# liuyuan-pal/NeuRay

Measured on AMD Instinct MI355X. Metric: rays/sec (64 coarse+32 fine samples), lego 800x800 synthetic, higher is better.
Workload: dtype fp32 (MLP contractions: operands split exactly into 3 bf16 parts, 6 bf16-MFMA products per K = 32, fp32 accumulate); 1 GPU; lego-800 synthetic (nerf_synthetic/lego/black_800 shape): 800x800 = 640000 rays/image, 8 ref views, 64 coarse + 32 fine samples, maps 200x200x32, 1 image per step per GPU; ray_batch=65536, parallelism=images sharded over 1 GPU(s), no collective

## Files before the change

__graft_entry__.py:

```python
import os
import subprocess
import sys

ROOT = os.path.dirname(os.path.abspath(__file__))
if ROOT not in sys.path:
    sys.path.insert(0, ROOT)


def build():
    from concurrent.futures import ThreadPoolExecutor
    from neuray_amd import build as nbuild
    sys.path.insert(0, os.path.join(ROOT, 'tests', 'emu'))
    import build_emu
    with ThreadPoolExecutor(4) as pool:
        jobs = [pool.submit(nbuild.build, False, True)]
        jobs += [pool.submit(build_emu.build, False, variant) for variant in ('fp32', 'bf16', 'bf16x3')]
        for j in jobs:
            j.result()
    from neuray_amd import _lib
    lib = _lib.bind(_lib.LIB_PATH)
    assert lib.neuray_abi_version() == 11 and lib.neuray_is_device_build() == 1 and lib.neuray_operand_precision() == 32
    import neuray_amd.network.renderer


def smoke():
    import numpy as np
    import torch
    from oracle import neuray_oracle as orc
    from neuray_amd.network.renderer import NeuralRayBaseRenderer

    assert torch.cuda.is_available(), "smoke() needs the MI355X"
    dev = 'cuda:0'
    cfg = {'use_hierarchical_sampling': True, 'dist_decoder_cfg': {'use_vis': False}, 'depth_sample_num': 32,
           'fine_depth_sample_num': 32, 'agg_net_cfg': {'sample_num': 32}, 'fine_agg_net_cfg': {'sample_num': 32}}
    torch.manual_seed(0)
    r = NeuralRayBaseRenderer(cfg).eval()
    weights = {k: v.detach().numpy().copy() for k, v in r.state_dict().items()}
    r = r.to(dev)
    que, ref = orc.make_scene(96, 128, 4, seed=7)
    rng = np.random.RandomState(7)
    que['coords'] = (rng.rand(1, 96, 2) * np.array([127, 95])).astype(np.float32)
    tq = {k: torch.from_numpy(v).to(dev) for k, v in que.items()}
    tr = {k: torch.from_numpy(v).to(dev) for k, v in ref.items()}
    with torch.no_grad():
        got = r.render_impl(tq, tr, False)
    torch.cuda.synchronize()
    ocfg = dict(cfg, coarse_use_vis=False, fine_use_vis=True)
    want = orc.render_impl(weights, ocfg, dict(que, Ks_inv=torch.inverse(torch.from_numpy(que['Ks'])).numpy()), ref)
    err_c = float(np.abs(got['pixel_colors_nr'].cpu().numpy() - want['pixel_colors_nr']).max())
# ... 59 lines not shown
```

include/neuray_hip.h:

```cpp
#ifndef NEURAY_HIP_H
#define NEURAY_HIP_H

#include <stddef.h>

#ifdef __cplusplus
extern "C" {
#endif

#define NEURAY_ABI_VERSION 11
#define NEURAY_POINT_REC 20
#define NEURAY_VIEW_CONST 20
#define NEURAY_QUERY_CONST 28
#define NEURAY_PASS_TENSORS 68
#define NEURAY_DBG_FIELDS 16
#define NEURAY_MAX_VIEWS 16
#define NEURAY_MAX_SAMPLES 128

int neuray_abi_version(void);
const char* neuray_last_error(void);
int neuray_is_device_build(void);
int neuray_operand_precision(void);

size_t neuray_packed_pass_floats(void);
int neuray_pack_pass_weights(const float* const* tensors_host, float* packed_host);
// ... 223 lines not shown
long long neuray_lpips_head_workspace_bytes(int n, int h, int w);
int neuray_lpips_head(const float* f0_dev, const float* f1_dev, const float* lin_dev, int n, int f1_stride, int c, int h, int w,
                      void* workspace_dev, double* out_dev, int out_stride, void* stream);

#define NEURAY_LOSS_RENDER 0
#define NEURAY_LOSS_CONSIST 1
#define NEURAY_LOSS_DEPTH 2
#define NEURAY_LOSS_MAX_TERMS 4
typedef struct NeurayLossTerm {
    const float* pred_dev;
    const float* ref_dev;
    const void* mask_dev;
    const void* coords_dev;
    const float* range_dev;
    const float* grad_out_dev;
    float* d_pred_dev;
    int kind, rows, n, inner, stride, h, w, coords_i64, mask_u8, smooth_l1;
    float beta, thresh;
} NeurayLossTerm;
typedef struct NeurayTrainLossArgs {
    const NeurayLossTerm* terms;
    float* value_dev;
    double* den_dev;
    void* workspace_dev;
    int n_terms, reserved;
} NeurayTrainLossArgs;
long long neuray_train_loss_workspace_bytes(const NeurayLossTerm* terms, int n_terms);
int neuray_train_loss(const NeurayTrainLossArgs* args, void* stream);
int neuray_train_loss_backward(const NeurayTrainLossArgs* args, void* stream);

int neuray_mfma_selftest(const float* A_dev, const float* B_dev, float* D_dev, void* stream);
int neuray_group_sum_selftest(const float* x_dev, float* y_dev, void* stream);
int neuray_group_scatter_selftest(const float* x_dev, float* y_dev, void* stream);

int neuray_x3_selftest(const float* A_dev, const float* B_dev, float* D_dev, float* parts_dev, void* stream);
int neuray_points_resident_workgroups(int arith, int rfn);

#ifdef __cplusplus
}
#endif
#endif
```

neuray_amd/_lib.py:

```python
import ctypes as C
import os

import torch

HERE = os.path.dirname(os.path.abspath(__file__))
LIB_PATH = os.environ.get('NEURAY_HIP_LIB', os.path.join(HERE, 'libneuray_hip.so'))
BF16_LIB_PATH = os.path.join(HERE, 'libneuray_hip_bf16.so')
BF16X3_LIB_PATH = os.path.join(HERE, 'libneuray_hip_bf16x3.so')

PASS_TENSORS = 68
POINT_REC = 20
VIEW_CONST = 20
QUERY_CONST = 28
DBG_FIELDS = 16
MAX_VIEWS = 16
MAX_SAMPLES = 128
MAX_BACKWARD_SAMPLES = 128

ARITH_F32, ARITH_X3 = 0, 1

c_float_p = C.POINTER(C.c_float)


class NeurayPointsArgs(C.Structure):
# ... 107 lines not shown
    'neuray_inorm_backward': (C.c_int, [C.c_void_p, C.c_void_p, C.c_longlong, C.c_void_p, C.c_longlong, C.c_void_p, C.c_void_p] + [C.c_int] * 6 + [C.c_void_p] * 6),
    'neuray_upsample2x_pad_forward': (C.c_int, [C.c_void_p, C.c_int, C.c_int, C.c_int, C.c_int, C.c_float, C.c_float, C.c_void_p, C.c_void_p]),
    'neuray_upsample2x_pad_backward': (C.c_int, [C.c_void_p, C.c_int, C.c_int, C.c_int, C.c_int, C.c_void_p, C.c_void_p, C.c_void_p, C.c_void_p,
                                                 C.c_void_p, C.c_void_p, C.c_void_p, C.c_void_p]),
    'neuray_direct_render_points': (C.c_int, [C.c_void_p] * 7 + [C.c_int] * 5 + [C.c_float, C.c_void_p, C.c_void_p, C.c_void_p]),
    'neuray_direct_render_rays': (C.c_int, [C.c_void_p, C.c_void_p, C.c_int, C.c_int, C.c_int, C.c_int, C.c_void_p, C.c_void_p, C.c_void_p]),
    'neuray_direct_render_rays_backward': (C.c_int, [C.c_void_p] * 4 + [C.c_int] * 2 + [C.c_void_p] * 3),
    'neuray_direct_render_points_backward': (C.c_int, [C.c_void_p] * 9 + [C.c_int] * 6 + [C.c_void_p] * 2),
    'neuray_dist_decoder_rows': (C.c_int, [C.c_void_p, C.c_void_p, C.c_int, C.c_int, C.c_float, C.c_void_p, C.c_void_p, C.c_void_p,
                                           C.c_void_p, C.c_void_p]),
    'neuray_self_hit_prob': (C.c_int, [C.c_void_p, C.c_void_p, C.c_void_p, C.c_void_p, C.c_void_p, C.c_void_p, C.c_int, C.c_int,
                                       C.c_void_p, C.c_void_p]),
    'neuray_mfma_selftest': (C.c_int, [C.c_void_p, C.c_void_p, C.c_void_p, C.c_void_p]),
    'neuray_x3_selftest': (C.c_int, [C.c_void_p, C.c_void_p, C.c_void_p, C.c_void_p, C.c_void_p]),
    'neuray_points_resident_workgroups': (C.c_int, [C.c_int, C.c_int]),
    'neuray_render_rays_backward': (C.c_int, [C.POINTER(NeurayRaysBwdArgs), C.c_void_p]),
    'neuray_flat_pass_floats': (C.c_size_t, []),
    'neuray_flat_tensor_offset': (C.c_size_t, [C.c_int]),
    'neuray_packed_t_floats': (C.c_size_t, []),
    'neuray_pack_pass_t_index_map': (C.c_int, [C.c_int, C.c_void_p]),
    'neuray_points_backward_handover_floats': (C.c_size_t, [C.c_int]),
    'neuray_packed_quad_ranges': (C.c_int, [C.c_int, C.c_void_p, C.c_int]),
    'neuray_render_points_backward': (C.c_int, [C.POINTER(NeurayPointsBwdArgs), C.c_void_p]),
    'neuray_self_hit_prob_backward': (C.c_int, [C.c_void_p, C.c_void_p, C.c_void_p, C.c_void_p, C.c_void_p, C.c_int, C.c_int,
                                                         C.c_float, C.c_void_p, C.c_int, C.c_int, C.c_void_p, C.c_void_p, C.c_void_p]),
    'neuray_dist_decoder_rows_backward': (C.c_int, [C.c_void_p, C.c_void_p, C.c_void_p, C.c_int, C.c_int, C.c_float, C.c_void_p, C.c_void_p,
                                                           C.c_void_p, C.c_void_p, C.c_void_p, C.c_void_p, C.c_void_p]),
    'neuray_interpolate_feats_backward_staged': (C.c_int, [C.c_void_p, C.c_void_p, C.c_void_p, C.c_int, C.c_int, C.c_int, C.c_int, C.c_int, C.c_int,
                                                         C.c_int, C.c_int, C.c_void_p, C.c_void_p, C.c_void_p]),
    'neuray_interpolate_feats_backward': (C.c_int, [C.c_void_p, C.c_void_p, C.c_void_p, C.c_int, C.c_int, C.c_int, C.c_int,
                                                    C.c_int, C.c_int, C.c_int, C.c_int, C.c_void_p, C.c_void_p]),
    'neuray_group_sum_selftest': (C.c_int, [C.c_void_p, C.c_void_p, C.c_void_p]),
    'neuray_group_scatter_selftest': (C.c_int, [C.c_void_p, C.c_void_p, C.c_void_p]),
    'neuray_warp_variance': (C.c_int, [C.c_void_p, C.c_void_p, C.c_void_p, C.c_void_p, C.c_void_p, C.c_int, C.c_int, C.c_int, C.c_int, C.c_int,
                                       C.c_int, C.c_void_p, C.c_void_p]),
    'neuray_warp_variance_layout': (C.c_int, [C.c_void_p, C.c_void_p, C.c_void_p, C.c_void_p, C.c_void_p, C.c_int, C.c_int, C.c_int, C.c_int, C.c_int,
                                              C.c_int, C.c_int, C.c_void_p, C.c_void_p]),
    'neuray_conv3d_c32_c8': (C.c_int, [C.c_void_p, C.c_void_p, C.c_void_p, C.c_float, C.c_int, C.c_int, C.c_int, C.c_int, C.c_void_p, C.c_void_p]),
    'neuray_convtranspose3d_bn_leaky': (C.c_int, [C.c_void_p, C.c_void_p, C.c_void_p, C.c_float, C.c_void_p, C.c_int, C.c_int, C.c_int, C.c_int, C.c_int,
                                                C.c_int, C.c_void_p, C.c_void_p]),
    'neuray_conv3d_bn_leaky': (C.c_int, [C.c_void_p, C.c_void_p, C.c_void_p, C.c_float, C.c_int, C.c_int, C.c_int, C.c_int, C.c_int, C.c_int, C.c_int,
                                       C.c_void_p, C.c_void_p]),
    'neuray_conv3x3_x3_pack_bytes': (C.c_longlong, [C.c_int, C.c_int]),
    'neuray_conv3x3_x3_pack': (C.c_int, [C.c_void_p, C.c_int, C.c_int, C.c_void_p, C.c_void_p, C.c_void_p]),
    'neuray_conv3x3_x3': (C.c_int, [C.c_void_p, C.c_void_p, C.c_void_p, C.c_int, C.c_int, C.c_int, C.c_int, C.c_int, C.c_int, C.c_void_p, C.c_void_p]),
    'neuray_conv3x3_x3_relu': (C.c_int, [C.c_void_p, C.c_void_p, C.c_void_p, C.c_int, C.c_int, C.c_int, C.c_int, C.c_int, C.c_int, C.c_void_p, C.c_void_p]),
    'neuray_conv3x3_x3_wrw_workspace_floats': (C.c_longlong, [C.c_int, C.c_int, C.c_int, C.c_int, C.c_int]),
    'neuray_conv3x3_x3_wrw': (C.c_int, [C.c_void_p, C.c_void_p, C.c_int, C.c_int, C.c_int, C.c_int, C.c_int, C.c_void_p, C.c_void_p, C.c_void_p]),
    'neuray_scale_shift_leaky': (C.c_int, [C.c_void_p, C.c_void_p, C.c_void_p, C.c_int, C.c_int, C.c_longlong, C.c_float, C.c_void_p]),
    'neuray_conv3d_c8_c1': (C.c_int, [C.c_void_p, C.c_void_p, C.c_float, C.c_int, C.c_int, C.c_int, C.c_int, C.c_void_p, C.c_void_p]),
    'neuray_convtranspose3d_c16_c8': (C.c_int, [C.c_void_p, C.c_void_p, C.c_void_p, C.c_float, C.c_void_p, C.c_int, C.c_int, C.c_int, C.c_int, C.c_void_p, C.c_void_p]),
    'neuray_diff_feats': (C.c_int, [C.c_void_p, C.c_void_p, C.c_void_p, C.c_int, C.c_int, C.c_int, C.c_void_p, C.c_void_p]),
    'neuray_image_metrics_workspace_bytes': (C.c_longlong, [C.c_int, C.c_int, C.c_int]),
    'neuray_image_metrics': (C.c_int, [C.POINTER(NeurayImageMetricsArgs), C.c_void_p]),
    'neuray_lpips_stem': (C.c_int, [C.c_void_p, C.c_int, C.POINTER(C.c_float), C.POINTER(C.c_float), C.c_void_p, C.c_void_p, C.c_int, C.c_int, C.c_int,
                                    C.c_int, C.c_void_p, C.c_void_p]),
    'neuray_maxpool2x2': (C.c_int, [C.c_void_p, C.c_longlong, C.c_int, C.c_int, C.c_void_p, C.c_void_p]),
    'neuray_lpips_head_workspace_bytes': (C.c_longlong, [C.c_int, C.c_int, C.c_int]),
    'neuray_lpips_head': (C.c_int, [C.c_void_p, C.c_void_p, C.c_void_p, C.c_int, C.c_int, C.c_int, C.c_int, C.c_int, C.c_void_p, C.c_void_p, C.c_int,
                                    C.c_void_p]),
    'neuray_train_loss_workspace_bytes': (C.c_longlong, [C.POINTER(NeurayLossTerm), C.c_int]),
    'neuray_train_loss': (C.c_int, [C.POINTER(NeurayTrainLossArgs), C.c_void_p]),
    'neuray_train_loss_backward': (C.c_int, [C.POINTER(NeurayTrainLossArgs), C.c_void_p]),
}


# ... 36 lines not shown
```

neuray_amd/build.py:

```python
import os
import subprocess
import sys

HERE = os.path.dirname(os.path.abspath(__file__))
CSRC = os.path.join(HERE, 'csrc')
OUT = os.path.join(HERE, 'libneuray_hip.so')
SOURCES = [os.path.join(CSRC, 'neuray_hip.hip'), os.path.join(CSRC, 'nr_pack.cpp')]
DEPS = SOURCES + [os.path.join(CSRC, f) for f in ('nr_kernels.h', 'nr_kernels_bwd.h', 'nr_kernels_bwd2.h', 'nr_kernels_dr.h', 'nr_kernels_norm.h', 'nr_kernels_conv3d.h', 'nr_kernels_conv2d.h', 'nr_kernels_metrics.h', 'nr_kernels_loss.h', 'nr_kernels_lpips.h', 'nr_device.h', 'nr_layout.h', 'nr_platform.h', 'nr_pack.h')] + \
    [os.path.join(os.path.dirname(HERE), 'include', 'neuray_hip.h')]
HIPCC = os.environ.get('HIPCC', '/opt/rocm/bin/hipcc')
FLAGS = ['--offload-arch=gfx950', '-O3', '-std=c++17', '-fPIC', '-shared', '-ffp-contract=off', '-Wno-unused-value', '-Wno-pass-failed',
         '-Wno-comment']


OUT_BF16 = os.path.join(HERE, 'libneuray_hip_bf16.so')
OUT_BF16X3 = os.path.join(HERE, 'libneuray_hip_bf16x3.so')


def needs_build(out=OUT):
    return not os.path.exists(out) or any(os.path.getmtime(out) < os.path.getmtime(d) for d in DEPS)


def build(force=False, verbose=False):
    jobs = []
    for out, extra in ((OUT, []), (OUT_BF16, ['-DNR_BF16_QUADS']), (OUT_BF16X3, ['-DNR_BF16_QUADS', '-DNR_BF16_SPLIT'])):
        if not force and not needs_build(out):
            continue
        tmp = out + '.building'
        cmd = [HIPCC] + FLAGS + extra + SOURCES + ['-o', tmp]
        if verbose:
            print(' '.join(cmd[:-1] + [out]))
        jobs.append((out, tmp, cmd, subprocess.Popen(cmd)))
    failed = []
    for out, tmp, cmd, proc in jobs:
        if proc.wait() == 0:
            os.replace(tmp, out)
        else:
            failed.append(cmd)
            if os.path.exists(tmp):
                os.remove(tmp)
    if failed:
        raise subprocess.CalledProcessError(1, failed[0])
    return OUT


if __name__ == '__main__':
    print(build(force='-f' in sys.argv, verbose=True))
```

neuray_amd/csrc/neuray_hip.hip:

```cpp
#include "nr_kernels.h"
#include "nr_kernels_bwd.h"
#include "nr_kernels_norm.h"
#include "nr_kernels_conv3d.h"
#include "nr_kernels_conv2d.h"
#include "nr_kernels_metrics.h"
#include "nr_kernels_loss.h"
#include "nr_kernels_lpips.h"
#if defined(NR_BF16_QUADS) && !defined(NR_BF16_SPLIT)
#define NR_INFERENCE_ONLY 1
#else
#include "nr_kernels_bwd2.h"
#endif
#include "nr_kernels_dr.h"
#include "nr_pack.h"
#include "../../include/neuray_hip.h"

#include <cmath>
#include <cstdarg>
#include <cstdio>
#include <cstring>
#include <cstdlib>

namespace {

// ... 857 lines not shown
    if (has_vis_head && d_vis) NR_LAUNCH(nr::decoder_rows_backward2_kernel<true>, grid, dim3(64), 0, stream, p);
    else NR_LAUNCH(nr::decoder_rows_backward2_kernel<false>, grid, dim3(64), 0, stream, p);
    return check_launch("neuray_dist_decoder_rows_backward");
#endif
}

int neuray_interpolate_feats_backward(const float* d_out, const float* points, const float* mask, int b, int n, int c, int fh,
                                      int fw, int h_full, int w_full, int align_corners, float* d_feats, void* stream) {
    if (!d_out || !points || !d_feats) return fail("neuray_interpolate_feats_backward: null argument");
    if (b < 1 || n < 1 || c < 1 || fh < 1 || fw < 1) return fail("neuray_interpolate_feats_backward: bad shape");
    NR_LAUNCH(nr::interpolate_backward_kernel, dim3(grid_for((long long)b * n * c, 256, 4096)), dim3(256), 0, stream, d_out, points,
              mask, b, n, c, fh, fw, h_full, w_full, align_corners, d_feats);
    return check_launch("neuray_interpolate_feats_backward");
}

int neuray_interpolate_feats_backward_staged(const float* d_out, const float* points, const float* mask, int b, int n, int c, int fh,
                                             int fw, int h_full, int w_full, int align_corners, float* tmp_nhwc_zeroed, float* d_feats, void* stream) {
    if (!d_out || !points || !d_feats || !tmp_nhwc_zeroed) return fail("neuray_interpolate_feats_backward_staged: null argument");
    if (b < 1 || n < 1 || c < 1 || fh < 1 || fw < 1 || (long long)b * ((c + 31) / 32) > 65535) return fail("neuray_interpolate_feats_backward_staged: bad shape");
    NR_LAUNCH(nr::interpolate_backward_nhwc_kernel, dim3(grid_for((long long)b * n * c, 256, 4096)), dim3(256), 0, stream, d_out, points,
              mask, b, n, c, fh, fw, h_full, w_full, align_corners, tmp_nhwc_zeroed);
    if (int rc = check_launch("neuray_interpolate_feats_backward_staged")) return rc;
    NR_LAUNCH(nr::nhwc_add_to_nchw_kernel, dim3((fh * fw + 31) / 32, ((c + 31) / 32) * b), dim3(256), 0, stream, tmp_nhwc_zeroed, fh * fw, c, d_feats);
    return check_launch("neuray_interpolate_feats_backward_staged");
}

int neuray_group_sum_selftest(const float* x, float* y, void* stream) {
    NR_LAUNCH(nr::group_sum_selftest_kernel, dim3(1), dim3(64), 0, stream, x, y);
    return check_launch("neuray_group_sum_selftest");
}
int neuray_group_scatter_selftest(const float* x, float* y, void* stream) {
    NR_LAUNCH(nr::group_scatter_selftest_kernel, dim3(1), dim3(64), 0, stream, x, y);
    return check_launch("neuray_group_scatter_selftest");
}

static void metrics_tiles(int y0, int y1, int x0, int x1, int& tiles_y, int& tiles_x) {
    tiles_y = (y1 - y0 - (nr::kMetWin - 1) + nr::kMetTH - 1) / nr::kMetTH;
    tiles_x = (x1 - x0 - (nr::kMetWin - 1) + nr::kMetTW - 1) / nr::kMetTW;
}

long long neuray_image_metrics_workspace_bytes(int n, int h, int w) {
    if (n < 1 || h < nr::kMetWin || w < nr::kMetWin) return -1;
    int ty, tx;
    metrics_tiles(0, h, 0, w, ty, tx);
    return (long long)n * ty * tx * nr::kMetPartial * 8;
}

int neuray_image_metrics(const NeurayImageMetricsArgs* a, void* stream) {
    if (!a) return fail("neuray_image_metrics: null args");
    if (!a->pred_dev || !a->gt_dev || !a->sse_dev || !a->ssim_dev || !a->workspace_dev) return fail("neuray_image_metrics: missing array");
    if (a->n < 1 || a->h < 1 || a->w < 1 || a->gt_stride < 0) return fail("neuray_image_metrics: bad shape n=%d h=%d w=%d gt_stride=%d", a->n, a->h, a->w, a->gt_stride);
    if (a->variant != NEURAY_SSIM_BOX11 && a->variant != NEURAY_SSIM_GAUSS11) return fail("neuray_image_metrics: unknown SSIM variant %d", a->variant);
    if (a->roi_y0 < 0 || a->roi_x0 < 0 || a->roi_y1 > a->h || a->roi_x1 > a->w || a->roi_y0 >= a->roi_y1 || a->roi_x0 >= a->roi_x1)
        return fail("neuray_image_metrics: region [%d, %d) x [%d, %d) is not inside the %d x %d image", a->roi_y0, a->roi_y1, a->roi_x0, a->roi_x1, a->h, a->w);
    if (a->roi_y1 - a->roi_y0 < nr::kMetWin || a->roi_x1 - a->roi_x0 < nr::kMetWin)
        return fail("neuray_image_metrics: the %d x %d region is smaller than the 11 x 11 SSIM window", a->roi_y1 - a->roi_y0, a->roi_x1 - a->roi_x0);
    nr::MetricsParams p;
    p.pred = a->pred_dev; p.gt = a->gt_dev; p.quant = a->quant_dev; p.sse = a->sse_dev; p.ssim = a->ssim_dev;
    p.ws = static_cast<double*>(a->workspace_dev);
    p.n = a->n; p.gt_stride = a->gt_stride; p.u8 = a->input_u8 ? 1 : 0; p.h = a->h; p.w = a->w;
    p.y0 = a->roi_y0; p.y1 = a->roi_y1; p.x0 = a->roi_x0; p.x1 = a->roi_x1;
    metrics_tiles(p.y0, p.y1, p.x0, p.x1, p.tiles_y, p.tiles_x);
    double sum = 0.0;
    for (int k = 0; k < nr::kMetWin; ++k) {
        const double d = k - (nr::kMetWin - 1) / 2;
        p.taps[k] = std::exp(-0.5 * d * d / (1.5 * 1.5));
// ... 149 lines not shown
```

neuray_amd/csrc/nr_kernels.h:

```cpp
#pragma once
#include "nr_device.h"

namespace nr {

__global__ void view_setup_kernel(const float* __restrict__ poses, const float* __restrict__ Ks,
                                  const float* __restrict__ depth_range, int n, float* __restrict__ out) {
    const int v = blockIdx.x * blockDim.x + threadIdx.x;
    if (v >= n) return;
    const float* P = poses + v * 12;
    const float* K = Ks + v * 9;
    float* o = out + v * kViewConst;
    for (int i = 0; i < 3; ++i)
        for (int j = 0; j < 4; ++j)
            o[i * 4 + j] = dot3(K[i * 3 + 0], K[i * 3 + 1], K[i * 3 + 2], P[j], P[4 + j], P[8 + j]);
    for (int i = 0; i < 3; ++i) o[12 + i] = dot3(-P[i], -P[4 + i], -P[8 + i], P[3], P[7], P[11]);
    o[15] = rn_div(-1.0f, depth_range[2 * v]);
    o[16] = rn_div(-1.0f, depth_range[2 * v + 1]);
    o[17] = rn_div(1.0f, rn_sub(o[16], o[15]));
    o[18] = 0.0f; o[19] = 0.0f;
}

__global__ void query_setup_kernel(const float* __restrict__ pose, const float* __restrict__ Kinv,
                                   const float* __restrict__ depth_range, float* __restrict__ o) {
    if (blockIdx.x * blockDim.x + threadIdx.x != 0) return;
// ... 117 lines not shown
        const int mo = wave + j * nw;
        if (mo < 4) {
            mfma_quad<NT>(r.q[j][2 * STAT], 0, xq, accg[j]);
            mfma_quad<NT>(r.q[j][2 * STAT + 1], 1, xq, accg[j]);
            NR_PRAGMA_UNROLL
            for (int t = 0; t < NT; ++t) accg[j][t] = nr_mfma16(r.s1[j][STAT], x1[t][0], accg[j][t]);
        }
    }
}

template <int NA, int IDLE, int R, int RMAX, int OP>
__device__ __forceinline__ void view_allreduce(const float (&v)[NA > 0 ? NA : 1][R], float (&out)[R], float* red, int wave,
                                               int nw, int lane) {
    NR_PRAGMA_UNROLL
    for (int r = 0; r < R; ++r) {
        const bool is_max = OP == RED_MAX || (OP == RED_MAX0 && r == 0);
        float a = NA > 0 ? v[0][r] : (is_max ? -1e9f : 0.0f);
        NR_PRAGMA_UNROLL
        for (int s = 1; s < NA; ++s) a = red_combine<OP, R>(a, v[s][r], r);
        if (IDLE > 0 && NA > 0 && is_max) a = fmaxf(a, -1e9f);
        out[r] = a;
    }
    block_allreduce<R, RMAX, OP, R>(out, red, wave, nw, lane);
}

template <int N> struct SlotCount { static constexpr int value = N; };

#ifndef NR_POINT_SKIP
#define NR_POINT_SKIP 1
#endif
#ifndef NR_POINT_TILE_ORDER
#define NR_POINT_TILE_ORDER 0
#endif
#ifndef NR_POINT_TRANSPOSED
#define NR_POINT_TRANSPOSED 1
#endif

template <int NT, int VPW, bool HAS_VIS, int OWN, int MAXT, int MINW, bool SAVE = false, bool DBG = false, int AR = AR_F32>
__global__ void __launch_bounds__(MAXT, MINW) points_kernel(PointParams p) {
    static_assert(NT == 1, "one 16-point tile per wave iteration");
    static_assert(AR == AR_F32 || !SAVE, "the training forward runs on the fp32 MFMA");
    NR_DYNAMIC_SMEM(float, smem);
    constexpr int RMAX = point_rmax<NT>();
    constexpr int NS = VPW;
    constexpr bool SKIP = (NR_POINT_SKIP != 0) && !SAVE && !DBG && VPW == 2;
    const int lane = threadIdx.x & 63;
    const int wave = NR_UNIFORM((int)(threadIdx.x >> 6));
    const int nw = (p.rfn + VPW - 1) / VPW;
    const int g = lane >> 4, c = lane & 15;
    float* red = smem;
    float* xch = smem + (size_t)(nw + 1) * RMAX * 64;
    float* wl = xch + (AR == AR_X3 ? 0 : 16 * NT * 64);
    auto xrow = [&](int mo, int r) -> float* {
        if constexpr (AR == AR_X3 && OWN == 1) return red + ((size_t)mo * RMAX + r) * 64;
        else if constexpr (AR == AR_X3) return red + ((size_t)(mo % nw) * RMAX + (mo / nw) * 4 + r) * 64;
        else return xch + (mo * 4 + r) * 64;
    };
    auto make_w = [&]() {
        if constexpr (AR == AR_X3) return GlbW3{nr_make_wbuf(p.weights, sizeof(float) * kPackedPointFloatsX3)};
        else return nr_make_wbuf(p.weights, sizeof(float) * kPackedPassFloats);
    };
    const auto W = make_w();
    const float w_m1 = (float)(p.w - 1), h_m1 = (float)(p.h - 1);
    const float inv_w_m1 = 1.0f / w_m1, inv_h_m1 = 1.0f / h_m1, inv_rfn = 1.0f / (float)p.rfn;
    const size_t fmap = (size_t)p.fh * p.fw * 32, imap = (size_t)p.h * p.w * 4;
    const nr_mbuf rf_map = nr_make_mbuf(p.ray_feats, sizeof(float) * fmap * p.rfn);
    const nr_mbuf if_map = nr_make_mbuf(p.img_feats, sizeof(float) * fmap * p.rfn);
    const nr_mbuf rgb_map = nr_make_mbuf(p.rgba, sizeof(float) * imap * p.rfn);
    const int goff = 32 * g;
    const int npts = p.rn * p.dn;
    const int dn = p.dn;
    const bool use_vis = p.use_vis != 0;
    const bool folded = AR == AR_X3 || (!SAVE && p.folded != 0);
    const int bid = (int)(blockIdx.x % 8) * (int)(gridDim.x / 8) + (int)(blockIdx.x / 8);
    int seq0 = 0;
#ifndef NR_X3_BG_RESIDENT
#define NR_X3_BG_RESIDENT 1
#endif
#ifndef NR_X3_GF_PREFETCH
#define NR_X3_GF_PREFETCH 1
#endif
    constexpr bool BG_RES = AR == AR_X3 && OWN == 1 && (NR_X3_BG_RESIDENT != 0);
    BgResident<OWN> bgres;
    if constexpr (BG_RES) bg_resident_load(W, lane, wave, nw, bgres);
    int n_active = 0, n_slots = 0;
    constexpr bool TR = (NR_POINT_TRANSPOSED != 0) && !SAVE && !DBG;
    const int nloop = TR ? ((p.rn + 15) / 16) * dn * 16 : npts;
#ifndef NR_POINT_CHUNK
#define NR_POINT_CHUNK 1
#endif
    constexpr int CH = NR_POINT_CHUNK;
    const int G = (int)gridDim.x;
    auto tile_base = [&](int it) { return (((it / CH) * G + bid) * CH + (it % CH)) * 16; };
    if (tile_base(0) < nloop) stage_issue<PH_DIST_M>(wl, W, wave, nw, lane);
    for (int it = 0, base; (base = tile_base(it)) < nloop; ++it, seq0 += phase_count(HAS_VIS)) {
        const bool more = tile_base(it + 1) < nloop;
        const int glane = lane + nr_opaque_zero();
#ifndef NR_NO_OPAQUE_WAVE
        const int wave_t = wave + nr_opaque_szero();
#else
        const int wave_t = wave;
#endif
        const int gg = glane >> 4;
        const bool dbg_lane = DBG && (gg == 0);
        const auto* pt = NR_ARGS_HERE(PointParams, p);
        int pidx; bool pvalid;
        float mask[NS], dlt[NS][4], tref[NS], pu[NS], pv[NS], lo, hi;
        int soff_f[NS], soff_c[NS];
        {
            int pi, ray, smp;
            const float* __restrict__ qc = pt->que_const;
            const float qnearp = qc[24], qfarp = qc[25], qinv = qc[27];
            const int dn = pt->dn, npts = pt->rn * dn;
            if constexpr (TR) {
#if NR_POINT_TILE_ORDER == 1
                const int tix = base >> 4, nrb = (pt->rn + 15) / 16;
                smp = tix / nrb;
                const int rb = tix - smp * nrb;
#else
                const int tix = base >> 4, rb = tix / dn;
                smp = tix - rb * dn;
#endif
                ray = rb * 16 + c;
                pvalid = ray < pt->rn;
                ray = pvalid ? ray : pt->rn - 1;
                pi = ray * dn + smp;
            } else {
                pi = base + c;
                pvalid = pi < npts;
                pi = pi < npts ? pi : npts - 1;
                ray = pi / dn;
                smp = pi - ray * dn;
            }
            pidx = pi;
            const Ray r = make_ray<false>(qc, pt->coords[2 * ray], pt->coords[2 * ray + 1]);
            const float* drow = pt->depth + (size_t)ray * dn;
            const float d = drow[smp];
            float s_c, s_n, s_p, s_x;
            {
                const int nxt = smp + 1 < dn ? smp + 1 : smp, prv = smp > 0 ? smp - 1 : 0;
                const float dg = drow[gg == 0 ? smp : (gg == 1 ? nxt : prv)];
                nr_group_gather4(norm_inv_depth_fast(dg, qnearp, qfarp, qinv), s_c, s_n, s_p, s_x);
            }
            const float half_c = (smp == dn - 1) ? 500000.0f : (s_n - s_c) * 0.5f;
            const float half_p = (s_c - s_p) * 0.5f;
            hi = half_c;
            lo = (smp == 0) ? half_c : half_p;
            const float px = rn_add(r.cx, rn_mul(r.dx, d));
            const float py = rn_add(r.cy, rn_mul(r.dy, d));
            const float pz = rn_add(r.cz, rn_mul(r.dz, d));
            NR_PRAGMA_UNROLL
            for (int s = 0; s < NS; ++s) {
                const int vraw = wave_t * VPW + s;
                const bool vok = vraw < pt->rfn;
                const int view = vok ? vraw : pt->rfn - 1;
                const float* __restrict__ vc = pt->view_const + view * kViewConst;
                Proj pr = project_point<false>(vc, px, py, pz, (float)pt->w, (float)pt->h);
                if (!vok) pr.mask = 0.0f;
                mask[s] = pr.mask;
                dlt[s][0] = pr.dirx - r.qx; dlt[s][1] = pr.diry - r.qy; dlt[s][2] = pr.dirz - r.qz;
                dlt[s][3] = dot3(pr.dirx, pr.diry, pr.dirz, r.qx, r.qy, r.qz);
                tref[s] = norm_inv_depth_fast(fmaxf(pr.z, 1e-5f), vc[15], vc[16], vc[17]);
                pu[s] = pr.u; pv[s] = pr.v;
                if (dbg_lane && pvalid && vok) {
                    float* d_ = pt->dbg + ((size_t)pi * pt->rfn + view) * kDbgFields;
                    d_[0] = pr.mask; d_[1] = pr.u; d_[2] = pr.v; d_[3] = pr.z;
                }
                soff_f[s] = view * (int)(fmap * sizeof(float)); soff_c[s] = view * (int)(imap * sizeof(float));
            }
        }

        auto tile = [&](auto na_tag) NR_LAMBDA_INLINE {
            constexpr int NA = decltype(na_tag)::value, NA1 = NA > 0 ? NA : 1, IDLE = NS - NA;
            constexpr bool SC = NA == 2 && !SAVE;
            float fray[NA1][8], fimg[NA1][8], rgb[NA1][3];
#ifdef NR_PROBE_PRE
            float fm1[NA1][8], fv1[NA1][8], fa1[NA1][8];
#endif
            if constexpr (NA > 0) {
                Taps tfs[NA], tcs[NA];
                NR_PRAGMA_UNROLL
                for (int s = 0; s < NA; ++s) {
                    tfs[s] = make_taps_fast(pu[s], pv[s], w_m1, h_m1, inv_w_m1, inv_h_m1, p.fw, p.fh, p.fw == p.w && p.fh == p.h);
                    tcs[s] = make_taps_fast(pu[s], pv[s], w_m1, h_m1, inv_w_m1, inv_h_m1, p.w, p.h, true);
#ifdef NR_PROBE_NO_GATHER
                    tfs[s].o00 = tfs[s].o10 = tfs[s].o01 = tfs[s].o11 = 0;
                    tcs[s].o00 = tcs[s].o10 = tcs[s].o01 = tcs[s].o11 = 0;
#endif
                }
                NR_PRAGMA_UNROLL
                for (int s = 0; s < NA; ++s) {
                    float4 qf[8], qi[8], qc4[4];
                    issue8(rf_map, goff, soff_f[s], tfs[s], qf);
                    issue8(if_map, goff, soff_f[s], tfs[s], qi);
                    issue_rgb(rgb_map, soff_c[s], tcs[s], qc4);
                    NR_PIN();
                    blend8(qf, tfs[s], mask[s], fray[s]);
                    blend8(qi, tfs[s], mask[s], fimg[s]);
                    blend_rgb(qc4, tcs[s], mask[s], rgb[s]);
                    NR_PRAGMA_UNROLL
                    for (int k = 0; k < 8; ++k) { NR_KEEP(fray[s][k]); NR_KEEP(fimg[s][k]); }
                    NR_PRAGMA_UNROLL
                    for (int j = 0; j < 3; ++j) NR_KEEP(rgb[s][j]);
                    NR_PIN();
#ifdef NR_PROBE_PRE
                    {
                        float4 q1[8], q2[8], q3[8];
                        issue8(rf_map, goff, soff_f[s] + 4096, tfs[s], q1);
                        issue8(rf_map, goff, soff_f[s] + 8192, tfs[s], q2);
                        issue8(rf_map, goff, soff_f[s] + 12288, tfs[s], q3);
                        NR_PIN();
                        blend8(q1, tfs[s], mask[s], fm1[s]);
                        blend8(q2, tfs[s], mask[s], fv1[s]);
                        blend8(q3, tfs[s], mask[s], fa1[s]);
                        NR_PRAGMA_UNROLL
                        for (int k = 0; k < 8; ++k) { NR_KEEP(fm1[s][k]); NR_KEEP(fv1[s][k]); NR_KEEP(fa1[s][k]); }
                        NR_PIN();
                    }
#endif
                }
            }
            float none[NA1][1];
            NR_PRAGMA_UNROLL
            for (int s = 0; s < NA1; ++s) none[s][0] = 0.0f;
            NoLayer last;
            decltype(auto) o_fray = operand<AR>(fray);
            decltype(auto) o_none = operand<AR>(none);

            float hit[NA1], vis[NA1];
            {
                float h1[NA1][8], h2[NA1][8], fm[NA1][2], fv[NA1][2], fa[NA1][1];
                float mu0[NA1], mu1[NA1], s0[NA1], s1[NA1], aw[NA1], nu[NA1];
// ... 541 lines not shown
                nonet[0][0] = 0.0f;
                NR_PRAGMA_UNROLL
                for (int k = 0; k < 16; ++k) h[0][k] = xrow(k >> 2, k & 3)[lane];
                layer_fwd<L_GF2, NT, ACT_ELU>(W, glane, h, nonet, G);
                if (pvalid)
                    *reinterpret_cast<float4*>(pt->point_out + (size_t)pidx * kPointRec + 4 * g) = make_float4(G[0][0], G[0][1], G[0][2], G[0][3]);
                if constexpr (SAVE) {
                    NR_PRAGMA_UNROLL
                    for (int r = 0; r < 4; ++r) p.saved[(size_t)(base / 16) * kSavedTileFloats + (kSavedGRow + r) * 64 + lane] = G[0][r];
                }
            }
            if (wave_t == (nw > 1 ? 1 : 0) && gg == 0) {
                if (pvalid)
                    *reinterpret_cast<float4*>(pt->point_out + (size_t)pidx * kPointRec + 16) = make_float4(big[9], big[10], big[11], msum);
            }
        };

        if constexpr (SKIP) {
            const bool a0 = __ballot(mask[0] != 0.0f) != 0ull, a1 = __ballot(mask[1] != 0.0f) != 0ull;
#ifdef NR_FORCE_NA
#ifdef NR_FORCE_NA_CONST
            const int na = NR_FORCE_NA;
#else
            const int na = NR_FORCE_NA + (p.rn < 0 ? (a0 ? 1 : 0) + (a1 ? 1 : 0) : 0);
#endif
#else
            const int na = (a0 ? 1 : 0) + (a1 ? 1 : 0);
#endif
            n_active += na; n_slots += NS;
            if (na == 2) {
                tile(SlotCount<2>{});
            } else if (na == 1) {
                if (!a0) {
                    mask[0] = mask[1]; tref[0] = tref[1]; pu[0] = pu[1]; pv[0] = pv[1]; soff_f[0] = soff_f[1]; soff_c[0] = soff_c[1];
                    NR_PRAGMA_UNROLL
                    for (int k = 0; k < 4; ++k) dlt[0][k] = dlt[1][k];
                }
                tile(SlotCount<1>{});
            } else {
                tile(SlotCount<0>{});
            }
        } else {
            tile(SlotCount<NS>{});
        }
    }
    if constexpr (SKIP) {
        if (p.slot_stats) {
            NR_BLOCK_SYNC();
            if (lane == 0) { red[2 * wave] = (float)n_active; red[2 * wave + 1] = (float)n_slots; }
            NR_BLOCK_SYNC();
            if (threadIdx.x == 0) {
                float a = 0.0f, b = 0.0f;
                for (int w = 0; w < nw; ++w) { a += red[2 * w]; b += red[2 * w + 1]; }
                atomicAdd(p.slot_stats, (unsigned long long)a);
                atomicAdd(p.slot_stats + 1, (unsigned long long)b);
            }
        }
    }
}

struct RayParams {
    const float* point_rec;
    const float* depth;
    const float* pos_enc;
    const float* weights;
    float* hit_prob;
    float* pixel;
// ... 670 lines not shown
                                   float* __restrict__ parts) {
    const int lane = threadIdx.x & 63, c = lane & 15, g = lane >> 4;
    float av[1][8], bv[1][8];
    for (int i = 0; i < 8; ++i) { av[0][i] = A[c * 32 + 8 * g + i]; bv[0][i] = B[(8 * g + i) * 16 + c]; }
    const Opnd3<1, 8> a3 = split_operand(av), b3 = split_operand(bv);
    Frag3 f;
    for (int pt = 0; pt < 3; ++pt)
        for (int i = 0; i < 4; ++i) f.p[pt][i] = a3.p[pt][0][i];
    v4f acc[1];
    acc[0][0] = 0.0f; acc[0][1] = 0.0f; acc[0][2] = 0.0f; acc[0][3] = 0.0f;
    mfma_unit3<L_DM1, 1>(f, 0, b3, acc);
    for (int r = 0; r < 4; ++r) D[(4 * g + r) * 16 + c] = acc[0][r];
    if (parts)
        for (int pt = 0; pt < 3; ++pt)
            for (int i = 0; i < 8; ++i) {
                const unsigned w = a3.p[pt][0][i / 2], u = (i & 1) ? (w & 0xffff0000u) : (w << 16);
                parts[(pt * 16 + c) * 32 + 8 * g + i] = __int_as_float((int)u);
            }
}

__global__ void group_sum_selftest_kernel(const float* __restrict__ x, float* __restrict__ y) {
    y[threadIdx.x & 63] = nr_group_sum(x[threadIdx.x & 63]);
}

__global__ void group_scatter_selftest_kernel(const float* __restrict__ x, float* __restrict__ y) {
    const int l = threadIdx.x & 63;
    const float s4 = nr_group_scatter4(x[l], x[64 + l], x[128 + l], x[192 + l]);
    float a, b, c, d, e, f;
    nr_group_gather4(s4, a, b, c, d);
    nr_group_gather2(nr_group_scatter2(x[l], x[64 + l]), e, f);
    y[l] = a; y[64 + l] = b; y[128 + l] = c; y[192 + l] = d; y[256 + l] = e; y[320 + l] = f; y[384 + l] = s4;
}

}
```

neuray_amd/csrc/nr_platform.h:

```cpp
#pragma once

#ifdef NEURAY_EMU
#include "hip_emu.h"
#define NR_UNIFORM(x) (x)
#define NR_GLOBAL_PTR(T) T*
#define NR_TO_GLOBAL(T, p) (p)
#define NR_FROM_GLOBAL(T, p) (p)
static inline float4 nr_gld4(const float* p) { return *reinterpret_cast<const float4*>(p); }
static inline void nr_gst4(float* p, float4 v) { *reinterpret_cast<float4*>(p) = v; }
#define NR_PRAGMA_UNROLL
#define NR_PRAGMA_UNROLL4
#define NR_LAMBDA_INLINE
#else
#include <hip/hip_runtime.h>

typedef float v4f __attribute__((ext_vector_type(4)));

__device__ __forceinline__ v4f nr_mfma16(float a, float b, v4f c) {
    return __builtin_amdgcn_mfma_f32_16x16x4f32(a, b, c, 0, 0, 0);
}
#ifdef NR_BF16_QUADS
typedef short nr_v4s __attribute__((ext_vector_type(4)));
typedef __bf16 nr_v2bf __attribute__((ext_vector_type(2)));
__device__ __forceinline__ unsigned nr_pk_bf16(float lo, float hi) {
// ... 268 lines not shown
    return r.x + r.y;
}
__device__ __forceinline__ float nr_group_scatter2(float a, float b) {
    typedef unsigned int v2u __attribute__((ext_vector_type(2)));
    typedef float v2f __attribute__((ext_vector_type(2)));
    const v2f p = __builtin_bit_cast(v2f, (v2u)__builtin_amdgcn_permlane16_swap(__builtin_bit_cast(unsigned, a), __builtin_bit_cast(unsigned, b), false, false));
    const unsigned s = __builtin_bit_cast(unsigned, p.x + p.y);
    const v2f r = __builtin_bit_cast(v2f, (v2u)__builtin_amdgcn_permlane32_swap(s, s, false, false));
    return r.x + r.y;
}
__device__ __forceinline__ void nr_group_halves(float x, float& lo, float& hi) {
    typedef unsigned int v2u __attribute__((ext_vector_type(2)));
    typedef float v2f __attribute__((ext_vector_type(2)));
    const unsigned u = __builtin_bit_cast(unsigned, x);
    const v2f r = __builtin_bit_cast(v2f, (v2u)__builtin_amdgcn_permlane32_swap(u, u, false, false));
    lo = r.x; hi = r.y;
}
__device__ __forceinline__ void nr_group_gather2(float x, float& a, float& b) {
    typedef unsigned int v2u __attribute__((ext_vector_type(2)));
    typedef float v2f __attribute__((ext_vector_type(2)));
    const unsigned u = __builtin_bit_cast(unsigned, x);
    const v2f r = __builtin_bit_cast(v2f, (v2u)__builtin_amdgcn_permlane16_swap(u, u, false, false));
    a = r.x; b = r.y;
}
__device__ __forceinline__ void nr_group_gather4(float x, float& a, float& b, float& c, float& d) {
    float lo, hi;
    nr_group_halves(x, lo, hi);
    nr_group_gather2(lo, a, b);
    nr_group_gather2(hi, c, d);
}
#endif

#ifdef NEURAY_EMU
static inline float nr_row_from_left(float v, float edge) { const int l = emu::my_lane(); const float t = emu_shfl_f(v, (l & 15) ? l - 1 : l); return (l & 15) ? t : edge; }
static inline float nr_row_from_right(float v, float edge) { const int l = emu::my_lane(); const float t = emu_shfl_f(v, (l & 15) != 15 ? l + 1 : l); return (l & 15) != 15 ? t : edge; }
#else
__device__ __forceinline__ float nr_row_from_left(float v, float edge) {
    return __builtin_bit_cast(float, __builtin_amdgcn_update_dpp(__builtin_bit_cast(int, edge), __builtin_bit_cast(int, v), 0x111, 0xf, 0xf, false));
}
__device__ __forceinline__ float nr_row_from_right(float v, float edge) {
    return __builtin_bit_cast(float, __builtin_amdgcn_update_dpp(__builtin_bit_cast(int, edge), __builtin_bit_cast(int, v), 0x101, 0xf, 0xf, false));
}
#endif

namespace nr {
#ifdef NEURAY_EMU
__device__ __forceinline__ float rn_mul(float a, float b) { volatile float r = a * b; return r; }
__device__ __forceinline__ float rn_add(float a, float b) { volatile float r = a + b; return r; }
__device__ __forceinline__ float rn_sub(float a, float b) { volatile float r = a - b; return r; }
__device__ __forceinline__ float rn_div(float a, float b) { volatile float r = a / b; return r; }
__device__ __forceinline__ float rn_sqrt(float a) { return sqrtf(a); }
#else
#pragma clang fp contract(off)
__device__ __forceinline__ float rn_mul(float a, float b) { return a * b; }
__device__ __forceinline__ float rn_add(float a, float b) { return a + b; }
__device__ __forceinline__ float rn_sub(float a, float b) { return a - b; }
__device__ __forceinline__ float rn_div(float a, float b) { return a / b; }
__device__ __forceinline__ float rn_sqrt(float a) { return __builtin_sqrtf(a); }
#endif
}
```

Measured before the change: 3.332 million rays/s.

## Distribute per-view projection and tap setup across lane groups, gather via permlane

In the x3 point kernel with two views per wave, each 16-lane group now does one view's projection and one bilinear tap set (fine map or image), instead of every lane computing both views and both tap sets redundantly. The results go back to all lanes through permlane-based gather2/gather4 exchanges, and the mask is folded into the tap weights. View constants are read with vectorized buffer loads. This cuts redundant ALU work per point, but adds cross-lane permute traffic and keeps more tap registers live. A reference build with the scatter disabled and a gather selftest are also added.

```diff
diff --git a/__graft_entry__.py b/__graft_entry__.py
--- a/__graft_entry__.py
+++ b/__graft_entry__.py
@@ -12,9 +12,11 @@
     from neuray_amd import build as nbuild
     sys.path.insert(0, os.path.join(ROOT, 'tests', 'emu'))
     import build_emu
-    with ThreadPoolExecutor(4) as pool:
+    import build_emu_geom_ref
+    with ThreadPoolExecutor(5) as pool:
         jobs = [pool.submit(nbuild.build, False, True)]
         jobs += [pool.submit(build_emu.build, False, variant) for variant in ('fp32', 'bf16', 'bf16x3')]
+        jobs.append(pool.submit(build_emu_geom_ref.build))
         for j in jobs:
             j.result()
     from neuray_amd import _lib
diff --git a/include/neuray_hip.h b/include/neuray_hip.h
--- a/include/neuray_hip.h
+++ b/include/neuray_hip.h
@@ -279,6 +279,7 @@
 int neuray_mfma_selftest(const float* A_dev, const float* B_dev, float* D_dev, void* stream);
 int neuray_group_sum_selftest(const float* x_dev, float* y_dev, void* stream);
 int neuray_group_scatter_selftest(const float* x_dev, float* y_dev, void* stream);
+int neuray_group_gather_selftest(const int* x_dev, int* y_dev, void* stream);
 
 int neuray_x3_selftest(const float* A_dev, const float* B_dev, float* D_dev, float* parts_dev, void* stream);
 int neuray_points_resident_workgroups(int arith, int rfn);
diff --git a/neuray_amd/_lib.py b/neuray_amd/_lib.py
--- a/neuray_amd/_lib.py
+++ b/neuray_amd/_lib.py
@@ -163,6 +163,7 @@
                                                     C.c_int, C.c_int, C.c_int, C.c_int, C.c_void_p, C.c_void_p]),
     'neuray_group_sum_selftest': (C.c_int, [C.c_void_p, C.c_void_p, C.c_void_p]),
     'neuray_group_scatter_selftest': (C.c_int, [C.c_void_p, C.c_void_p, C.c_void_p]),
+    'neuray_group_gather_selftest': (C.c_int, [C.c_void_p, C.c_void_p, C.c_void_p]),
     'neuray_warp_variance': (C.c_int, [C.c_void_p, C.c_void_p, C.c_void_p, C.c_void_p, C.c_void_p, C.c_int, C.c_int, C.c_int, C.c_int, C.c_int,
                                        C.c_int, C.c_void_p, C.c_void_p]),
     'neuray_warp_variance_layout': (C.c_int, [C.c_void_p, C.c_void_p, C.c_void_p, C.c_void_p, C.c_void_p, C.c_int, C.c_int, C.c_int, C.c_int, C.c_int,
diff --git a/neuray_amd/build.py b/neuray_amd/build.py
--- a/neuray_amd/build.py
+++ b/neuray_amd/build.py
@@ -15,6 +15,7 @@
 
 OUT_BF16 = os.path.join(HERE, 'libneuray_hip_bf16.so')
 OUT_BF16X3 = os.path.join(HERE, 'libneuray_hip_bf16x3.so')
+OUT_GEOM_REF = os.path.join(HERE, 'libneuray_hip_geom_ref.so')
 
 
 def needs_build(out=OUT):
@@ -23,7 +24,8 @@
 
 def build(force=False, verbose=False):
     jobs = []
-    for out, extra in ((OUT, []), (OUT_BF16, ['-DNR_BF16_QUADS']), (OUT_BF16X3, ['-DNR_BF16_QUADS', '-DNR_BF16_SPLIT'])):
+    for out, extra in ((OUT, []), (OUT_BF16, ['-DNR_BF16_QUADS']), (OUT_BF16X3, ['-DNR_BF16_QUADS', '-DNR_BF16_SPLIT']),
+                       (OUT_GEOM_REF, ['-DNR_GEOM_SCATTER=0'])):
         if not force and not needs_build(out):
             continue
         tmp = out + '.building'
diff --git a/neuray_amd/csrc/neuray_hip.hip b/neuray_amd/csrc/neuray_hip.hip
--- a/neuray_amd/csrc/neuray_hip.hip
+++ b/neuray_amd/csrc/neuray_hip.hip
@@ -913,6 +913,10 @@
 int neuray_group_scatter_selftest(const float* x, float* y, void* stream) {
     NR_LAUNCH(nr::group_scatter_selftest_kernel, dim3(1), dim3(64), 0, stream, x, y);
     return check_launch("neuray_group_scatter_selftest");
+}
+int neuray_group_gather_selftest(const int* x, int* y, void* stream) {
+    NR_LAUNCH(nr::group_gather_selftest_kernel, dim3(1), dim3(64), 0, stream, x, y);
+    return check_launch("neuray_group_gather_selftest");
 }
 
 static void metrics_tiles(int y0, int y1, int x0, int x1, int& tiles_y, int& tiles_x) {
diff --git a/neuray_amd/csrc/nr_kernels.h b/neuray_amd/csrc/nr_kernels.h
--- a/neuray_amd/csrc/nr_kernels.h
+++ b/neuray_amd/csrc/nr_kernels.h
@@ -173,6 +173,9 @@
 #ifndef NR_POINT_TILE_ORDER
 #define NR_POINT_TILE_ORDER 0
 #endif
+#ifndef NR_GEOM_SCATTER
+#define NR_GEOM_SCATTER 1
+#endif
 #ifndef NR_POINT_TRANSPOSED
 #define NR_POINT_TRANSPOSED 1
 #endif
@@ -185,6 +188,7 @@
     constexpr int RMAX = point_rmax<NT>();
     constexpr int NS = VPW;
     constexpr bool SKIP = (NR_POINT_SKIP != 0) && !SAVE && !DBG && VPW == 2;
+    constexpr bool GS = (NR_GEOM_SCATTER != 0) && !SAVE && VPW == 2 && AR == AR_X3;
     const int lane = threadIdx.x & 63;
     const int wave = NR_UNIFORM((int)(threadIdx.x >> 6));
     const int nw = (p.rfn + VPW - 1) / VPW;
@@ -248,6 +252,7 @@
         int pidx; bool pvalid;
         float mask[NS], dlt[NS][4], tref[NS], pu[NS], pv[NS], lo, hi;
         int soff_f[NS], soff_c[NS];
+        Taps tfs[NS], tcs[NS];
         {
             int pi, ray, smp;
             const float* __restrict__ qc = pt->que_const;
@@ -293,21 +298,70 @@
             NR_PRAGMA_UNROLL
             for (int s = 0; s < NS; ++s) {
                 const int vraw = wave_t * VPW + s;
+                const int view = vraw < pt->rfn ? vraw : pt->rfn - 1;
+                soff_f[s] = view * (int)(fmap * sizeof(float)); soff_c[s] = view * (int)(imap * sizeof(float));
+            }
+            if constexpr (GS) {
+                const int vraw = wave_t * VPW + (gg & 1);
                 const bool vok = vraw < pt->rfn;
                 const int view = vok ? vraw : pt->rfn - 1;
-                const float* __restrict__ vc = pt->view_const + view * kViewConst;
+                static_assert(kViewConst == 20, "five 16-byte loads per view");
+                float vc[kViewConst];
+                {
+                    const nr_buf vb = nr_make_buf(pt->view_const, sizeof(float) * kViewConst * (size_t)pt->rfn);
+                    const int vo = view * (int)(kViewConst * sizeof(float));
+                    NR_PRAGMA_UNROLL
+                    for (int q = 0; q < kViewConst / 4; ++q) {
+                        const float4 t = nr_buf_ld4(vb, vo, 16 * q);
+                        vc[4 * q] = t.x; vc[4 * q + 1] = t.y; vc[4 * q + 2] = t.z; vc[4 * q + 3] = t.w;
+                    }
+                }
                 Proj pr = project_point<false>(vc, px, py, pz, (float)pt->w, (float)pt->h);
                 if (!vok) pr.mask = 0.0f;
-                mask[s] = pr.mask;
-                dlt[s][0] = pr.dirx - r.qx; dlt[s][1] = pr.diry - r.qy; dlt[s][2] = pr.dirz - r.qz;
-                dlt[s][3] = dot3(pr.dirx, pr.diry, pr.dirz, r.qx, r.qy, r.qz);
-                tref[s] = norm_inv_depth_fast(fmaxf(pr.z, 1e-5f), vc[15], vc[16], vc[17]);
-                pu[s] = pr.u; pv[s] = pr.v;
-                if (dbg_lane && pvalid && vok) {
+                const float d0 = pr.dirx - r.qx, d1 = pr.diry - r.qy, d2 = pr.dirz - r.qz;
+                const float d3 = dot3(pr.dirx, pr.diry, pr.dirz, r.qx, r.qy, r.qz);
+                const float tr = norm_inv_depth_fast(fmaxf(pr.z, 1e-5f), vc[15], vc[16], vc[17]);
+                if (DBG && gg < 2 && pvalid && vok) {
                     float* d_ = pt->dbg + ((size_t)pi * pt->rfn + view) * kDbgFields;
                     d_[0] = pr.mask; d_[1] = pr.u; d_[2] = pr.v; d_[3] = pr.z;
                 }
-                soff_f[s] = view * (int)(fmap * sizeof(float)); soff_c[s] = view * (int)(imap * sizeof(float));
+                nr_group_gather2(pr.mask, mask[0], mask[1]);
+                nr_group_gather2(tr, tref[0], tref[1]);
+                nr_group_gather2(d0, dlt[0][0], dlt[1][0]);
+                nr_group_gather2(d1, dlt[0][1], dlt[1][1]);
+                nr_group_gather2(d2, dlt[0][2], dlt[1][2]);
+                nr_group_gather2(d3, dlt[0][3], dlt[1][3]);
+                const bool img = gg >= 2;
+                Taps t = make_taps_fast(pr.u, pr.v, w_m1, h_m1, inv_w_m1, inv_h_m1, img ? pt->w : pt->fw, img ? pt->h : pt->fh,
+                                        img || (pt->fw == pt->w && pt->fh == pt->h));
+                t.w00 *= pr.mask; t.w10 *= pr.mask; t.w01 *= pr.mask; t.w11 *= pr.mask;
+                nr_group_gather4i(t.o00, tfs[0].o00, tfs[1].o00, tcs[0].o00, tcs[1].o00);
+                nr_group_gather4i(t.o10, tfs[0].o10, tfs[1].o10, tcs[0].o10, tcs[1].o10);
+                nr_group_gather4i(t.o01, tfs[0].o01, tfs[1].o01, tcs[0].o01, tcs[1].o01);
+                nr_group_gather4i(t.o11, tfs[0].o11, tfs[1].o11, tcs[0].o11, tcs[1].o11);
+                nr_group_gather4(t.w00, tfs[0].w00, tfs[1].w00, tcs[0].w00, tcs[1].w00);
+                nr_group_gather4(t.w10, tfs[0].w10, tfs[1].w10, tcs[0].w10, tcs[1].w10);
+                nr_group_gather4(t.w01, tfs[0].w01, tfs[1].w01, tcs[0].w01, tcs[1].w01);
+                nr_group_gather4(t.w11, tfs[0].w11, tfs[1].w11, tcs[0].w11, tcs[1].w11);
+            } else {
+                NR_PRAGMA_UNROLL
+                for (int s = 0; s < NS; ++s) {
+                    const int vraw = wave_t * VPW + s;
+                    const bool vok = vraw < pt->rfn;
+                    const int view = vok ? vraw : pt->rfn - 1;
+                    const float* __restrict__ vc = pt->view_const + view * kViewConst;
+                    Proj pr = project_point<false>(vc, px, py, pz, (float)pt->w, (float)pt->h);
+                    if (!vok) pr.mask = 0.0f;
+                    mask[s] = pr.mask;
+                    dlt[s][0] = pr.dirx - r.qx; dlt[s][1] = pr.diry - r.qy; dlt[s][2] = pr.dirz - r.qz;
+                    dlt[s][3] = dot3(pr.dirx, pr.diry, pr.dirz, r.qx, r.qy, r.qz);
+                    tref[s] = norm_inv_depth_fast(fmaxf(pr.z, 1e-5f), vc[15], vc[16], vc[17]);
+                    pu[s] = pr.u; pv[s] = pr.v;
+                    if (dbg_lane && pvalid && vok) {
+                        float* d_ = pt->dbg + ((size_t)pi * pt->rfn + view) * kDbgFields;
+                        d_[0] = pr.mask; d_[1] = pr.u; d_[2] = pr.v; d_[3] = pr.z;
+                    }
+                }
             }
         }
 
@@ -319,11 +373,12 @@
             float fm1[NA1][8], fv1[NA1][8], fa1[NA1][8];
 #endif
             if constexpr (NA > 0) {
-                Taps tfs[NA], tcs[NA];
                 NR_PRAGMA_UNROLL
                 for (int s = 0; s < NA; ++s) {
-                    tfs[s] = make_taps_fast(pu[s], pv[s], w_m1, h_m1, inv_w_m1, inv_h_m1, p.fw, p.fh, p.fw == p.w && p.fh == p.h);
-                    tcs[s] = make_taps_fast(pu[s], pv[s], w_m1, h_m1, inv_w_m1, inv_h_m1, p.w, p.h, true);
+                    if constexpr (!GS) {
+                        tfs[s] = make_taps_fast(pu[s], pv[s], w_m1, h_m1, inv_w_m1, inv_h_m1, p.fw, p.fh, p.fw == p.w && p.fh == p.h);
+                        tcs[s] = make_taps_fast(pu[s], pv[s], w_m1, h_m1, inv_w_m1, inv_h_m1, p.w, p.h, true);
+                    }
 #ifdef NR_PROBE_NO_GATHER
                     tfs[s].o00 = tfs[s].o10 = tfs[s].o01 = tfs[s].o11 = 0;
                     tcs[s].o00 = tcs[s].o10 = tcs[s].o01 = tcs[s].o11 = 0;
@@ -336,9 +391,10 @@
                     issue8(if_map, goff, soff_f[s], tfs[s], qi);
                     issue_rgb(rgb_map, soff_c[s], tcs[s], qc4);
                     NR_PIN();
-                    blend8(qf, tfs[s], mask[s], fray[s]);
-                    blend8(qi, tfs[s], mask[s], fimg[s]);
-                    blend_rgb(qc4, tcs[s], mask[s], rgb[s]);
+                    const float bm = GS ? 1.0f : mask[s];
+                    blend8(qf, tfs[s], bm, fray[s]);
+                    blend8(qi, tfs[s], bm, fimg[s]);
+                    blend_rgb(qc4, tcs[s], bm, rgb[s]);
                     NR_PRAGMA_UNROLL
                     for (int k = 0; k < 8; ++k) { NR_KEEP(fray[s][k]); NR_KEEP(fimg[s][k]); }
                     NR_PRAGMA_UNROLL
@@ -946,7 +1002,9 @@
                 tile(SlotCount<2>{});
             } else if (na == 1) {
                 if (!a0) {
-                    mask[0] = mask[1]; tref[0] = tref[1]; pu[0] = pu[1]; pv[0] = pv[1]; soff_f[0] = soff_f[1]; soff_c[0] = soff_c[1];
+                    mask[0] = mask[1]; tref[0] = tref[1]; soff_f[0] = soff_f[1]; soff_c[0] = soff_c[1];
+                    if constexpr (GS) { tfs[0] = tfs[1]; tcs[0] = tcs[1]; }
+                    else { pu[0] = pu[1]; pv[0] = pv[1]; }
                     NR_PRAGMA_UNROLL
                     for (int k = 0; k < 4; ++k) dlt[0][k] = dlt[1][k];
                 }
@@ -1683,4 +1741,17 @@
     y[l] = a; y[64 + l] = b; y[128 + l] = c; y[192 + l] = d; y[256 + l] = e; y[320 + l] = f; y[384 + l] = s4;
 }
 
-}
+__global__ void group_gather_selftest_kernel(const int* __restrict__ x, int* __restrict__ y) {
+    const int l = threadIdx.x & 63;
+    const int v = x[l];
+    int a, b, c, d;
+    nr_group_gather4i(v, a, b, c, d);
+    float fa, fb, fc, fd, ga, gb;
+    nr_group_gather4(__int_as_float(v), fa, fb, fc, fd);
+    nr_group_gather2(__int_as_float(v), ga, gb);
+    y[l] = a; y[64 + l] = b; y[128 + l] = c; y[192 + l] = d;
+    y[256 + l] = __float_as_int(fa); y[320 + l] = __float_as_int(fb); y[384 + l] = __float_as_int(fc); y[448 + l] = __float_as_int(fd);
+    y[512 + l] = __float_as_int(ga); y[576 + l] = __float_as_int(gb);
+}
+
+}
diff --git a/neuray_amd/csrc/nr_platform.h b/neuray_amd/csrc/nr_platform.h
--- a/neuray_amd/csrc/nr_platform.h
+++ b/neuray_amd/csrc/nr_platform.h
@@ -324,6 +324,19 @@
 #endif
 
 #ifdef NEURAY_EMU
+static inline void nr_group_gather4i(int x, int& a, int& b, int& c, int& d) {
+    const int col = emu::my_lane() & 15;
+    a = __shfl(x, col); b = __shfl(x, col + 16); c = __shfl(x, col + 32); d = __shfl(x, col + 48);
+}
+#else
+__device__ __forceinline__ void nr_group_gather4i(int x, int& a, int& b, int& c, int& d) {
+    float fa, fb, fc, fd;
+    nr_group_gather4(__builtin_bit_cast(float, x), fa, fb, fc, fd);
+    a = __builtin_bit_cast(int, fa); b = __builtin_bit_cast(int, fb); c = __builtin_bit_cast(int, fc); d = __builtin_bit_cast(int, fd);
+}
+#endif
+
+#ifdef NEURAY_EMU
 static inline float nr_row_from_left(float v, float edge) { const int l = emu::my_lane(); const float t = emu_shfl_f(v, (l & 15) ? l - 1 : l); return (l & 15) ? t : edge; }
 static inline float nr_row_from_right(float v, float edge) { const int l = emu::my_lane(); const float t = emu_shfl_f(v, (l & 15) != 15 ? l + 1 : l); return (l & 15) != 15 ? t : edge; }
 #else
```

Measured after the change: 3.362 million rays/s, median of 6. About the same (+0.9%).
